# mmwillet/TTS.cpp

Hardware: AMD Instinct MI355X
Metric: audio-seconds/sec (Parler-TTS-Mini fp16, greedy decode + DAC to 44.1 kHz PCM) (higher is better)
Workload: dtype f16

## Files before the change

include/tts_hip.h:

```cpp
#ifndef TTS_HIP_H
#define TTS_HIP_H

#include <stddef.h>
#include <stdint.h>

#ifdef __cplusplus
extern "C" {
#endif

enum tts_hip_type {
    TTS_HIP_F32  = 0,
    TTS_HIP_F16  = 1,
    TTS_HIP_Q4_0 = 2,
    TTS_HIP_Q5_0 = 6,
    TTS_HIP_Q8_0 = 8,
};

#define TTS_HIP_MAX_DAC_BLOCKS 8

typedef struct tts_hip_desc {
    uint32_t struct_size;
    uint32_t hidden_size;
    uint32_t n_layers;
    uint32_t n_attn_heads;
// ... 213 lines not shown
} tts_hip_snac_desc;
tts_hip_ctx *tts_hip_snac_create(int device, const tts_hip_snac_desc *desc);
int tts_hip_snac_decode(tts_hip_ctx *ctx, const uint32_t *codes, uint32_t T, const float *noise, float *pcm_out);
int tts_hip_snac_halo_frames(const tts_hip_snac_desc *desc);
int tts_hip_snac_decode_windows(tts_hip_ctx *ctx, const uint32_t *codes, const uint32_t *frames, const uint32_t *keep0, const uint32_t *keep1, uint32_t n,
                                const float *noise, float *pcm_out);
int tts_hip_snac_decode_windows_begin(tts_hip_ctx *ctx, const uint32_t *codes, const uint32_t *frames, const uint32_t *keep0, const uint32_t *keep1, uint32_t n,
                                      const float *noise, float *pcm_out);
int tts_hip_snac_decode_windows_end(tts_hip_ctx *ctx);

int tts_hip_dac_decode(tts_hip_ctx *ctx, const uint32_t *codes, uint32_t frames, float *pcm_out);
int tts_hip_dac_decode_batch(tts_hip_ctx *ctx, const uint32_t *codes, const uint32_t *frames, uint32_t n, float *pcm_out);
int tts_hip_dac_halo_frames(const tts_hip_desc *desc);
int tts_hip_dac_decode_windows(tts_hip_ctx *ctx, const uint32_t *codes, const uint32_t *frames, const uint32_t *keep0, const uint32_t *keep1,
                               uint32_t n, float *pcm_out);

int64_t tts_hip_debug_read(tts_hip_ctx *ctx, const char *what, float *out, size_t max_floats);
int     tts_hip_set_debug(tts_hip_ctx *ctx, int on);

enum tts_hip_kclass {
    TTS_HIP_K_EMBED = 0,
    TTS_HIP_K_LN = 1,
    TTS_HIP_K_GEMM_QKV = 2,
    TTS_HIP_K_ATTN_SELF = 3,
    TTS_HIP_K_GEMM_ATTN_OUT = 4,
    TTS_HIP_K_GEMM_CROSS_Q = 5,
    TTS_HIP_K_ATTN_CROSS = 6,
    TTS_HIP_K_GEMM_CROSS_OUT = 7,
    TTS_HIP_K_GEMM_FC1 = 8,
    TTS_HIP_K_GEMM_FC2 = 9,
// ... 39 lines not shown
```

tts.cpp_amd/csrc/shim_codec.hip:

```cpp
#include "shim_internal.h"

#include "dac_kernels.h"
#include "dac_b3_kernels.h"
#include "kokoro_kernels.h"

static int dac_snapshot(tts_hip_ctx *c, int stage, const float *dev, size_t C, size_t L, size_t LS) {
    if (!c->debug) return 0;
    HIPCHK(hipStreamSynchronize(c->stream));
    std::vector<float> &v = c->dac_dbg[stage];
    v.resize(C * L);
    HIPCHK(hipMemcpy2DAsync(v.data(), L * 4, dev, LS * 4, L * 4, C, hipMemcpyDeviceToHost, c->stream));
    HIPCHK(hipStreamSynchronize(c->stream));
    return 0;
}

#define CI32_K1 16
#ifndef CI32_T
#define CI32_T 8
#endif
#ifndef CI32_K7
#define CI32_K7 4
#endif
static int conv_tile(int cout, int K, int *CO_T, int *CI_T) {
    if (K != 7 && K != 1) return -1;
// ... 509 lines not shown
    ResUnitArgs a{};
    a.x = x; a.y = y; a.w = c->packed_ru.at(r.in_w);
    a.b7 = (const float *) (c->arena + r.in_b); a.b1 = (const float *) (c->arena + r.out_b);
    a.alpha_in = (const float *) (c->arena + r.in_alpha); a.alpha_mid = (const float *) (c->arena + r.out_alpha);
    a.L = LS; a.dil = dil; a.pad = 3 * dil; a.frames = bt.frames; a.mult = bt.mult;
    const double Lv = bt.tot_frames * bt.mult;
    CHK(prof_begin(c, TTS_HIP_K_DAC_RESUNIT, (2.0 * C * Lv + 8.0 * C * C) * 4, 2.0 * C * (double) C * 8 * Lv));
    if (c->dac_tap7) {
        if (C == 96) CHK((launch_resunit_t7<3, 3>(c, a, bt.n)));
        else CHK((launch_resunit_t7<6, 4>(c, a, bt.n)));
    } else if (C == 96) CHK((launch_resunit_t<3, 4, 3>(c, a, bt.n)));
    else CHK((launch_resunit_t<6, 2, 4>(c, a, bt.n)));
    return prof_end(c);
}

static int dac_decode_batch_on(tts_hip_ctx *c, const uint32_t *codes, const uint32_t *frames, uint32_t n, float *pcm_out);
static int dac_decode_batch(tts_hip_ctx *c, const uint32_t *codes, const uint32_t *frames, uint32_t n, float *pcm_out) {
    if (!c || !c->finalized || !c->has_dac) return set_err("tts_hip_dac_decode: context has no finalized DAC");
    if (!frames || !codes || !pcm_out) return set_err("tts_hip_dac_decode: null argument");
    const uint32_t G = (uint32_t) std::max(1, c->dac_group);
    size_t code_off = 0, pcm_off = 0;
    for (uint32_t g0 = 0; g0 < n; g0 += G) {
        const uint32_t m = std::min(G, n - g0);
        size_t fr = 0;
        for (uint32_t i = 0; i < m; i++) fr += frames[g0 + i];
        int rc;
        {
            std::lock_guard<std::mutex> lock(g_dac_pass_mutex[(unsigned) c->device % 64]);
            if (!c->dac_stream) {
                rc = dac_decode_batch_on(c, codes + code_off * c->d_ncb, frames + g0, m, pcm_out + pcm_off);
            } else {
                hipStream_t ar = c->stream;
                c->stream = c->dac_stream;
                rc = dac_decode_batch_on(c, codes + code_off * c->d_ncb, frames + g0, m, pcm_out + pcm_off);
                if (rc) (void) hipStreamSynchronize(c->stream);
                c->stream = ar;
            }
            if (rc) (void) hipStreamSynchronize(c->stream);
        }
        if (rc) return rc;
        code_off += fr;
        pcm_off += fr * (size_t) c->d_up;
    }
    return 0;
}

static int dac_decode_batch_on(tts_hip_ctx *c, const uint32_t *codes, const uint32_t *frames, uint32_t n, float *pcm_out) {
    if (!c->weights_present) return set_err("tts_hip_dac_decode: weights not present");
    if (!codes || !pcm_out || !frames) return set_err("tts_hip_dac_decode: null argument");
    HIPCHK(hipSetDevice(c->device));
    uint32_t Fmax = 0;
    size_t tot = 0;
    for (uint32_t i = 0; i < n; i++) {
        if (frames[i] > c->d.dac_max_frames) return set_err("tts_hip_dac_decode: %u frames > max %u", frames[i], c->d.dac_max_frames);
        Fmax = std::max(Fmax, frames[i]);
        tot += frames[i];
    }
    if (Fmax == 0) return 0;
    for (size_t i = 0; i < tot * c->d_ncb; i++)
        if (codes[i] >= (uint32_t) c->d_cbsize) return set_err("tts_hip_dac_decode: code %u >= codebook size %d", codes[i], c->d_cbsize);
    c->dac_dbg.clear();
    CHK(ensure_packed(c));
    const size_t need_frames = (size_t) n * Fmax;
    size_t need_elems = 0, pcm_elems = 0;
    {
        int Lq = (int) Fmax;
        need_elems = (size_t) std::max(c->d_latent, c->d_c0) * dac_row_stride(c, Lq);
        if (c->packed_p.count(c->d_initw)) need_elems = std::max(need_elems, ((size_t) c->d_latent * dac_row_stride(c, Lq) * 3 + 1) / 2);
        for (auto &b : c->dblocks) {
            need_elems = std::max(need_elems, (size_t) b.cin * dac_row_stride(c, Lq));
            Lq = (Lq - 1) * b.stride - 2 * b.padding + 2 * b.stride;
            need_elems = std::max(need_elems, (size_t) b.cout * dac_row_stride(c, Lq));
            if (c->packed_p.count(b.res[0].in_w)) need_elems = std::max(need_elems, ((size_t) b.cout * dac_row_stride(c, Lq) * 3 + 1) / 2);
        }
        need_elems *= n;
        pcm_elems = (size_t) n * dac_row_stride(c, Lq);
    }
    DacBuffers &B = g_dac_buffers[(unsigned) c->device % 64];
    if (!c->dac_buf_user) { c->dac_buf_user = true; B.users++; }
    if (need_frames * c->d_ncb > B.cap_codes || need_elems > B.dbuf_elems || pcm_elems > B.h_pcm_elems || (!c->packed_p.empty() && !B.dplanes)) {
        HIPCHK(hipStreamSynchronize(c->stream));
        const size_t want_elems = std::max(need_elems, B.dbuf_elems), want_codes = std::max(need_frames * c->d_ncb, B.cap_codes), want_pcm = std::max(pcm_elems, B.h_pcm_elems);
        auto drop = [&]() {
            for (int i = 0; i < 3; i++) { free_dev(B.dbuf[i]); B.dbuf[i] = nullptr; }
            free_dev(B.dplanes); B.dplanes = nullptr;
            free_dev(B.d_codes); B.d_codes = nullptr;
            if (B.h_pcm) { (void) hipHostFree(B.h_pcm); B.h_pcm = nullptr; }
            B.dbuf_elems = B.cap_codes = B.h_pcm_elems = 0;
        };
        drop();
        hipError_t e = hipSuccess;
        for (int i = 0; i < 3 && e == hipSuccess; i++) e = hipMalloc((void **) &B.dbuf[i], want_elems * 4);
        if (e == hipSuccess && !c->packed_p.empty()) e = hipMalloc((void **) &B.dplanes, want_elems * 4);
        if (e == hipSuccess) e = hipMalloc((void **) &B.d_codes, want_codes * 4);
        if (e == hipSuccess) e = hipHostMalloc((void **) &B.h_pcm, want_pcm * 4);
        if (e != hipSuccess) {
            drop();
            return set_err("tts_hip_dac_decode: codec buffers of %zu floats x %d + %zu ids: %s", want_elems, c->packed_p.empty() ? 3 : 4, want_codes, hipGetErrorString(e));
        }
        B.dbuf_elems = want_elems; B.cap_codes = want_codes; B.h_pcm_elems = want_pcm;
    }
    if (n > c->d_frames_cap) {
        free_dev(c->d_frames);
        HIPCHK(hipMalloc((void **) &c->d_frames, (size_t) n * 4));
        c->d_frames_cap = n;
    }
    HIPCHK(hipMemcpyAsync(c->d_frames, frames, (size_t) n * 4, hipMemcpyHostToDevice, c->stream));
    {
        size_t off = 0;
        for (uint32_t i = 0; i < n; i++) {
            if (frames[i]) HIPCHK(hipMemcpyAsync(B.d_codes + (size_t) i * Fmax * c->d_ncb, codes + off * c->d_ncb, (size_t) frames[i] * c->d_ncb * 4,
                                                 hipMemcpyHostToDevice, c->stream));
            off += frames[i];
        }
    }
    DacBatch bt;
    bt.n = (int) n; bt.frames = c->d_frames; bt.mult = 1; bt.tot_frames = (double) tot;
    int L = (int) Fmax;
    int LS = dac_row_stride(c, L);
    float *cur = B.dbuf[0], *t1 = B.dbuf[1], *t2 = B.dbuf[2];

    DacEmbedArgs ea{};
    ea.frames = c->d_frames;
    ea.codes = B.d_codes; ea.codebook = (const float *) (c->arena + c->d_codebook); ea.proj_w = (const float *) (c->arena + c->d_projw);
    ea.proj_b = (const float *) (c->arena + c->d_projb); ea.n_cb = c->d_ncb; ea.cb_size = c->d_cbsize; ea.cb_dim = c->d_cbdim;
    ea.latent = c->d_latent; ea.T = L; ea.Tout = LS; ea.out = cur; ea.x_f16 = c->dac_f16 ? 1 : 0;
    CHK(prof_begin(c, TTS_HIP_K_DAC_EMBED, (double) c->d_latent * tot * 4, 2.0 * c->d_latent * tot * c->d_ncb * c->d_cbdim));
    if (c->d_ncb == 9 && c->d_cbdim == 8)
        hipLaunchKernelGGL((dac_embed_tile_kernel<9, 8>), dim3((L + 63) / 64, (c->d_latent + 4 * EMB_CH - 1) / (4 * EMB_CH), n), dim3(256), 0, c->stream, ea);
    else
// ... 58 lines not shown
        for (int r = 0; r < 3; r++) {
            int dil = 1;
            for (int e = 0; e < r; e++) dil *= 3;
            if (resunit_fused(c, b.res[r], dil)) {
                CHK(launch_resunit(c, bt, b.res[r], C, LS, dil, cur, t1));
                std::swap(cur, t1);
                continue;
            }
            CHK(launch_conv(c, bt, cur, C, LS, b.res[r].in_w, b.res[r].in_b, b.res[r].in_alpha, true, C, 7, 3 * dil, dil, nullptr, false, t1,
                            b.res[r].out_alpha, true));
            CHK(launch_conv(c, bt, t1, C, LS, b.res[r].out_w, b.res[r].out_b, 0, false, C, 1, 0, 1, cur, false, t2));
            std::swap(cur, t2);
        }
        if (n == 1) CHK(dac_snapshot(c, 2 + (int) bi, cur, (size_t) C, (size_t) L, (size_t) LS));
    }
    CHK(launch_conv(c, bt, cur, C, LS, c->d_fw, c->d_fb, c->d_falpha, true, 1, 7, 3, 1, nullptr, true, t1));
    HIPCHK(hipMemcpyAsync(B.h_pcm, t1, (size_t) n * LS * 4, hipMemcpyDeviceToHost, c->stream));
    HIPCHK(hipStreamSynchronize(c->stream));
    size_t off = 0;
    for (uint32_t i = 0; i < n; i++) {
        memcpy(pcm_out + off, B.h_pcm + (size_t) i * LS, (size_t) frames[i] * c->d_up * 4);
        off += (size_t) frames[i] * c->d_up;
    }
    return 0;
}

extern "C" int tts_hip_dac_decode(tts_hip_ctx *c, const uint32_t *codes, uint32_t frames, float *pcm_out) {
    return dac_decode_batch(c, codes, &frames, 1, pcm_out);
}

extern "C" int tts_hip_dac_decode_batch(tts_hip_ctx *c, const uint32_t *codes, const uint32_t *frames, uint32_t n, float *pcm_out) {
    if (n == 0) return 0;
    return dac_decode_batch(c, codes, frames, n, pcm_out);
}

static int64_t floor_div(int64_t a, int64_t b) { return a >= 0 ? a / b : -((-a + b - 1) / b); }

extern "C" int tts_hip_dac_halo_frames(const tts_hip_desc *d) {
    if (!d) return set_err("tts_hip_dac_halo_frames: null desc");
// ... 841 lines not shown
```

tts.cpp_amd/csrc/shim_core.hip:

```cpp
#include "shim_internal.h"

static thread_local char g_err[1024] = "";
int set_err(const char *fmt, ...) {
    va_list ap;
    va_start(ap, fmt);
    vsnprintf(g_err, sizeof(g_err), fmt, ap);
    va_end(ap);
    return -1;
}

extern "C" const char *tts_hip_last_error(void) { return g_err; }
extern "C" const char *tts_hip_version(void) { return "tts_hip 0.1 (gfx950)"; }

static float h2f_host(uint16_t h) {
    const uint32_t sign = (uint32_t) (h & 0x8000u) << 16;
    uint32_t exp = (h >> 10) & 0x1F, man = h & 0x3FF, bits;
    if (exp == 0) {
        if (man == 0) bits = sign;
        else {
            exp = 113;
            while ((man & 0x400) == 0) { man <<= 1; exp--; }
            bits = sign | (exp << 23) | ((man & 0x3FF) << 13);
        }
    } else if (exp == 31) bits = sign | 0x7F800000u | (man << 13);
// ... 151 lines not shown
    else if (k == "b1_fc2_split") c->b1_fc2_split = v != 0;
    else if (k == "b1_defer_combine") c->b1_defer_combine = v != 0;
    else if (k == "b1_stamps") c->b1_stamps_want = v != 0;
    else return set_err("tts_hip_tune: unknown key '%s'", key);
    return 0;
}

void free_dev(void *p) { if (p) (void) hipFree(p); }
std::mutex g_dac_pass_mutex[64];
static void dac_buffers_release(tts_hip_ctx *c) {
    if (!c->dac_buf_user) return;
    std::lock_guard<std::mutex> lock(g_dac_pass_mutex[(unsigned) c->device % 64]);
    DacBuffers &B = g_dac_buffers[(unsigned) c->device % 64];
    c->dac_buf_user = false;
    if (--B.users > 0) return;
    for (int i = 0; i < 3; i++) { free_dev(B.dbuf[i]); B.dbuf[i] = nullptr; }
    free_dev(B.dplanes); B.dplanes = nullptr;
    free_dev(B.d_codes); B.d_codes = nullptr;
    if (B.h_pcm) { (void) hipHostFree(B.h_pcm); B.h_pcm = nullptr; }
    B.dbuf_elems = B.cap_codes = B.h_pcm_elems = 0;
    B.users = 0;
}

static std::mutex g_arena_mutex;
static std::map<void *, int> g_arena_refs;
void arena_own(tts_hip_ctx *c) { std::lock_guard<std::mutex> l(g_arena_mutex); g_arena_refs[c->arena] = 1; }
void arena_share(tts_hip_ctx *c) {
    std::lock_guard<std::mutex> l(g_arena_mutex);
    auto it = g_arena_refs.find(c->arena);
    c->arena_counted = it != g_arena_refs.end();
    if (c->arena_counted) it->second++;
}
void arena_release(tts_hip_ctx *c) {
    if (!c->arena) return;
    if (c->arena_external && !c->arena_counted) return;
// ... 21 lines not shown
                     c->di_xn, c->di_qkv, c->di_q, c->di_att, c->di_gu, c->di_g, c->di_parts, c->di_logits, c->di_guided})
        free_dev(p);
    for (uint32_t *p : {c->di_tok, c->di_epos, c->di_eseq, c->di_kbeg, c->di_kend, c->di_ids, c->di_pos, c->di_seq, c->di_cend, c->di_stok, c->di_loop, c->di_hist, c->di_look, c->di_sbud, c->di_sadm}) free_dev(p);
    free_dev(c->di_suni);
    free_dev(c->di_e16);
    for (int i = 0; i < 3; i++) free_dev(c->sbuf[i]);
    free_dev(c->s_in); free_dev(c->s_out);
    if (c->h_in) (void) hipHostFree(c->h_in);
    if (c->h_out) (void) hipHostFree(c->h_out);
    if (c->h_hist) (void) hipHostFree(c->h_hist);
    free_dev(c->ls.state); free_dev(c->ls.tokens); free_dev(c->ls.smp); free_dev(c->ls.uni); free_dev(c->ls.cand); free_dev(c->ls.total);
    if (c->ls.h_state) (void) hipHostFree(c->ls.h_state);
    free_dev(c->t5_bucket); free_dev(c->t5_x); free_dev(c->t5_qkv); free_dev(c->t5_att); free_dev(c->t5_ug); free_dev(c->t5_g); free_dev(c->t5_y); free_dev(c->t5_ids); free_dev(c->logits); free_dev(c->part); free_dev(c->attn_cnt); free_dev(c->b1_stamps); free_dev(c->dbg); free_dev(c->d_ids); free_dev(c->d_pos);
    free_dev(c->d_seq); free_dev(c->d_gather); free_dev(c->d_tok); free_dev(c->d_step); free_dev(c->d_steps_done); free_dev(c->d_tokens_out);
    free_dev(c->d_eos); free_dev(c->d_frames);
    dac_buffers_release(c);
    for (auto &pw : c->packed) free_dev(pw.second);
    for (auto &pw : c->packed16) free_dev(pw.second);
    for (auto &pw : c->packed_b3) free_dev(pw.second);
    free_dev(c->cond_text_enc); free_dev(c->cond_cross_kv);
    for (auto &pw : c->packed_ru) free_dev(pw.second);
    for (auto &pw : c->packed_ct) free_dev(pw.second);
    for (auto &pw : c->packed_p) free_dev(pw.second);
    if (c->h_ids) (void) hipHostFree(c->h_ids);
    if (c->h_pos) (void) hipHostFree(c->h_pos);
    if (c->h_seq) (void) hipHostFree(c->h_seq);
    if (c->h_tok) (void) hipHostFree(c->h_tok);
    if (c->h_logits) (void) hipHostFree(c->h_logits);
    if (c->h_di) (void) hipHostFree(c->h_di);
    if (c->h_di_look) (void) hipHostFree(c->h_di_look);
// ... 654 lines not shown
```

tts.cpp_amd/csrc/shim_internal.h:

```cpp
#pragma once
#include "../../include/tts_hip.h"

#include <hip/hip_runtime.h>

#include <algorithm>
#include <atomic>
#include <cmath>
#include <cstdarg>
#include <cstdio>
#include <cstdlib>
#include <cstring>
#include <map>
#include <set>
#include <mutex>
#include <string>
#include <vector>

#include <unordered_map>
#define LLAMA_GREEDY_CHUNK 8

int set_err(const char *fmt, ...);
#define HIPCHK(expr)                                                                          \
    do {                                                                                      \
        hipError_t _e = (expr);                                                               \
// ... 39 lines not shown
struct DRes { size_t in_alpha, in_w, in_b, out_alpha, out_w, out_b; };
struct DBlock { int stride, padding, cin, cout; size_t alpha, w, b; DRes res[3]; };

struct CopyItem { size_t dst; std::string src; size_t src_off = 0; size_t bytes = 0; };

struct ProfEv { hipEvent_t a, b; int kclass; };

constexpr int GRAPH_KEY_ROWS = 8192;

struct DacBuffers {
    float *dbuf[3] = {nullptr, nullptr, nullptr};
    size_t dbuf_elems = 0;
    size_t cap_codes = 0;
    float *dplanes = nullptr;
    uint32_t *d_codes = nullptr;
    float *h_pcm = nullptr;
    size_t h_pcm_elems = 0;
    int users = 0;
};
extern DacBuffers g_dac_buffers[64];
extern std::mutex g_dac_pass_mutex[64];

struct tts_hip_ctx {
    int device = 0;
    hipStream_t stream = nullptr;
    hipStream_t dac_stream = nullptr;
    tts_hip_desc d{};
    std::map<std::string, Tensor> tensors;
    bool planned = false, finalized = false, weights_present = false;
    bool has_parler = false, has_dac = false;

    char *arena = nullptr;
    size_t arena_bytes = 0;
    bool arena_external = false;
// ... 182 lines not shown
        std::vector<uint32_t> start, row_utt;
    } gl;
    int gen_total = 0;
    bool gen_compact = true;
    uint32_t *d_tokens_out = nullptr;
    size_t tokens_out_cap = 0;
    uint8_t *d_eos = nullptr;
    uint32_t *h_ids = nullptr, *h_pos = nullptr, *h_seq = nullptr, *h_tok = nullptr;
    float *h_logits = nullptr;
    std::vector<uint32_t> host_pos;

    size_t dac_frame_elems = 0;
    size_t dac_cap_frames = 0;
    uint32_t *d_frames = nullptr;
    size_t d_frames_cap = 0;
    bool debug = false;
    std::map<int, std::vector<float>> dac_dbg;
    std::vector<float> win_pcm;
    std::map<size_t, float *> packed;
    std::set<size_t> packed_direct;
    std::map<size_t, _Float16 *> packed16;
    std::map<size_t, __bf16 *> packed_b3;
    std::map<size_t, __bf16 *> packed_ru;
    std::map<size_t, __bf16 *> packed_p;
    int dac_split = 1;
    int dac_f16_planes = 1;
    int dac_tap7 = 1;
    int dac_wdma = 1;
    int dac_planes = 1;
    bool dac_buf_user = false;
// ... 97 lines not shown
```

tts.cpp_amd/hip.py:

```python
import ctypes as C
import os

import numpy as np

from . import gguf

PKG_DIR = os.path.dirname(os.path.abspath(__file__))
MAX_DAC_BLOCKS = 8

FLAG_NO_GRAPH, FLAG_VALU_GEMM, FLAG_NO_DAC, FLAG_NO_PARLER, FLAG_DEQUANT_Q, FLAG_DAC_F32 = 1, 2, 4, 8, 16, 32
KCLASSES = ["embed", "ln", "gemm_qkv", "attn_self", "gemm_attn_out", "gemm_cross_q", "attn_cross", "gemm_cross_out", "gemm_fc1",
            "gemm_fc2", "gemm_heads", "sample", "gemm_other", "dac_embed", "dac_conv7", "dac_conv1", "dac_convt", "dac_final", "dac_resunit", "kokoro_conv_mfma"]


class HipError(RuntimeError):
    pass


class Desc(C.Structure):
    _fields_ = [
        ("struct_size", C.c_uint32),
        ("hidden_size", C.c_uint32), ("n_layers", C.c_uint32), ("n_attn_heads", C.c_uint32),
        ("n_output_heads", C.c_uint32), ("output_vocab_size", C.c_uint32), ("max_ctx_length", C.c_uint32),
        ("n_encode_length", C.c_uint32), ("use_cross_attn", C.c_uint32),
# ... 35 lines not shown
        (n, C.c_float) for n in ("attn_scale", "upsample_scale", "sample_rate", "sin_amp", "noise_std", "voice_threshold")] + [
        ("up_stride", C.c_uint32 * 4), ("up_padding", C.c_uint32 * 4), ("noise_stride", C.c_uint32 * 4), ("noise_padding", C.c_uint32 * 4),
        ("res_padding", (C.c_uint32 * 3) * 16), ("res_dilation", (C.c_uint32 * 3) * 16), ("noise_res_padding", (C.c_uint32 * 3) * 4),
        ("noise_res_dilation", (C.c_uint32 * 3) * 4), ("flags", C.c_uint32)]


class KStat(C.Structure):
    _fields_ = [("ms_total", C.c_double), ("launches", C.c_uint64), ("bytes_total", C.c_double), ("flops_total", C.c_double)]


EXPORTS = [
    "tts_hip_device_count", "tts_hip_create", "tts_hip_destroy", "tts_hip_last_error", "tts_hip_version",
    "tts_hip_upload", "tts_hip_arena_bytes", "tts_hip_finalize", "tts_hip_arena_ptr", "tts_hip_arena_filled",
    "tts_hip_parler_set_text_encoding", "tts_hip_parler_reset", "tts_hip_parler_prefill", "tts_hip_parler_prefill_batch", "tts_hip_parler_step",
    "tts_hip_parler_step_greedy", "tts_hip_parler_generate_greedy", "tts_hip_parler_generate_sampled", "tts_hip_sample_logits",
    "tts_hip_t5_create", "tts_hip_t5_encode", "tts_hip_t5_output_size", "tts_hip_snac_create", "tts_hip_snac_decode", "tts_hip_orpheus_create", "tts_hip_orpheus_decode", "tts_hip_orpheus_step_batch", "tts_hip_orpheus_generate_batch", "tts_hip_orpheus_generate_greedy", "tts_hip_orpheus_generate_sampled", "tts_hip_orpheus_sample_logits", "tts_hip_dia_create", "tts_hip_dia_encode", "tts_hip_dia_step", "tts_hip_dia_encode_slot", "tts_hip_dia_step_batch", "tts_hip_dia_generate", "tts_hip_kokoro_create", "tts_hip_kokoro_durations", "tts_hip_kokoro_generate", "tts_hip_dac_decode", "tts_hip_dac_decode_batch", "tts_hip_debug_read",
    "tts_hip_set_debug", "tts_hip_profile", "tts_hip_profile_get", "tts_hip_kclass_name", "tts_hip_stream",
    "tts_hip_synchronize", "tts_hip_dac_arith", "tts_hip_broadcast_weights", "tts_hip_comm_unique_id", "tts_hip_broadcast_weights_rank", "tts_hip_tune",
    "tts_hip_parler_stream_begin", "tts_hip_parler_stream_admit", "tts_hip_parler_stream_run", "tts_hip_parler_stream_collect", "tts_hip_parler_stream_end",
    "tts_hip_parler_gen_begin", "tts_hip_parler_gen_launch", "tts_hip_parler_gen_wait", "tts_hip_dac_halo_frames", "tts_hip_dac_decode_windows",
    "tts_hip_snac_halo_frames", "tts_hip_snac_decode_windows", "tts_hip_snac_decode_windows_begin", "tts_hip_snac_decode_windows_end",
    "tts_hip_orpheus_gen_begin", "tts_hip_orpheus_gen_launch", "tts_hip_orpheus_gen_wait",
    "tts_hip_orpheus_stream_begin", "tts_hip_orpheus_stream_admit", "tts_hip_orpheus_stream_run", "tts_hip_orpheus_stream_collect", "tts_hip_orpheus_stream_end",
    "tts_hip_orpheus_sample_logits_rows",
    "tts_hip_orpheus_stream_begin_mixed", "tts_hip_orpheus_stream_admit_mixed", "tts_hip_orpheus_sample_logits_rows_mixed",
    "tts_hip_dia_gen_begin", "tts_hip_dia_gen_launch", "tts_hip_dia_gen_wait",
    "tts_hip_dia_stream_begin", "tts_hip_dia_stream_admit", "tts_hip_dia_stream_run", "tts_hip_dia_stream_collect", "tts_hip_dia_stream_end",
    "tts_hip_dia_stream_launch", "tts_hip_dia_stream_wait", "tts_hip_dia_stream_drop",
]

class Sampling(C.Structure):
# ... 59 lines not shown
    L.tts_hip_dia_create.argtypes = [C.c_int, C.POINTER(DiaDesc)]
    L.tts_hip_dia_encode.argtypes = [vp, u32p, C.c_uint32, f32p]
    L.tts_hip_dia_step.argtypes = [vp, u32p, C.c_uint32, f32p, f32p]
    L.tts_hip_dia_encode_slot.argtypes = [vp, C.c_uint32, u32p, C.c_uint32, f32p]
    L.tts_hip_dia_step_batch.argtypes = [vp, C.c_uint32, u32p, u32p, u32p, f32p, f32p]
    L.tts_hip_dia_generate.argtypes = [vp, C.c_uint32, C.c_uint32, C.POINTER(DiaCodes), C.POINTER(Sampling), f32p, u32p, u32p]
    L.tts_hip_snac_create.restype = vp
    L.tts_hip_snac_create.argtypes = [C.c_int, C.POINTER(SnacDesc)]
    L.tts_hip_snac_decode.argtypes = [vp, u32p, C.c_uint32, f32p, f32p]
    L.tts_hip_t5_create.restype = vp
    L.tts_hip_t5_create.argtypes = [C.c_int, C.POINTER(T5Desc)]
    L.tts_hip_t5_encode.argtypes = [vp, u32p, C.c_uint32, f32p]
    L.tts_hip_t5_output_size.argtypes = [vp]
    L.tts_hip_dac_decode.argtypes = [vp, u32p, C.c_uint32, f32p]
    L.tts_hip_dac_decode_batch.argtypes = [vp, u32p, u32p, C.c_uint32, f32p]
    L.tts_hip_debug_read.argtypes = [vp, C.c_char_p, f32p, C.c_size_t]
    L.tts_hip_debug_read.restype = C.c_int64
    L.tts_hip_set_debug.argtypes = [vp, C.c_int]
    L.tts_hip_profile.argtypes = [vp, C.c_int]
    L.tts_hip_profile_get.argtypes = [vp, C.c_int, C.POINTER(KStat)]
    L.tts_hip_kclass_name.argtypes = [C.c_int]
    L.tts_hip_kclass_name.restype = C.c_char_p
    L.tts_hip_stream.argtypes = [vp]
    L.tts_hip_stream.restype = vp
    L.tts_hip_synchronize.argtypes = [vp]
    L.tts_hip_tune.argtypes = [vp, C.c_char_p, C.c_int]
    L.tts_hip_parler_stream_begin.argtypes = [vp, C.c_uint32, C.c_uint32, C.c_uint32, C.c_uint32, C.POINTER(Sampling)]
    L.tts_hip_parler_stream_admit.argtypes = [vp, C.c_uint32, u32p, u32p, u32p, f32p]
    L.tts_hip_parler_stream_run.argtypes = [vp, C.c_uint32, u32p, u32p, u32p]
    L.tts_hip_parler_stream_collect.argtypes = [vp, C.c_uint32, C.c_uint32, u32p]
# ... 927 lines not shown
```

tts.cpp_amd/host/parler_runner.cpp:

```cpp
#include "parler_runner.h"

#include <algorithm>
#include <cstdlib>
#include <cstring>

#include "gguf.h"

parler_model_loader::parler_model_loader() : tts_model_loader{"parler-tts"} {}
const parler_model_loader parler_loader{};
void parler_register() {}

static parler_hparams read_hparams(const gguf_file & m) {
    parler_hparams hp;
    if (!m.get_u32({"parler-tts.decoder.encode_length", "encode_length"}, hp.n_encode_length))
        TTS_ABORT("key 'parler-tts.decoder.encode_length' must be specified in gguf file.\n");
    m.get_u32({"parler-tts.decoder.hidden_size", "hidden_size"}, hp.hidden_size);
    m.get_u32({"parler-tts.decoder.output_heads", "output_heads"}, hp.n_output_heads);
    m.get_u32({"parler-tts.decoder.context_length", "ctx_length"}, hp.max_ctx_length);
    m.get_u32({"parler-tts.decoder.attention.head_count", "attn_heads"}, hp.n_attn_heads);
    m.get_u32({"parler-tts.decoder.out_vocab_size", "out_vocab_size"}, hp.output_vocab_size);
    m.get_u32({"parler-tts.decoder.audio_vocab_size", "audio_vocab_size"}, hp.audio_vocab_size);
    m.get_u32({"parler-tts.decoder.max_generation", "max_generation"}, hp.max_generation_size);
    m.get_u32({"parler-tts.decoder.num_hidden_layers", "num_hidden_layers"}, hp.n_layers);
    m.get_u32({"audio.bos_token_id", "bos_token_id"}, hp.bos_token_id);
// ... 343 lines not shown
                go = hook->emit();
            }
        }
    }
    if (hook && go) {
        finished.assign(n, true);
        hook->plan(toks, finished);
        (void) hook->emit();
    }
    return toks;
}

std::vector<tts_response> parler_runner::decode_frames(const std::vector<uint32_t> & codes, const std::vector<uint32_t> & frames) {
    size_t total = 0;
    for (uint32_t f : frames) total += (size_t) f * hp.up_sampling_factor;
    pcm.assign(total, 0.0f);
    if (total) hip_check(tts_hip_dac_decode_batch(ctx, codes.data(), frames.data(), (uint32_t) frames.size(), pcm.data()), "tts_hip_dac_decode_batch");
    std::vector<tts_response> audio(frames.size());
    size_t off = 0;
    for (size_t i = 0; i < frames.size(); i++) {
        audio[i].data = pcm.data() + off;
        audio[i].n_outputs = (size_t) frames[i] * hp.up_sampling_factor;
        off += audio[i].n_outputs;
    }
    return audio;
}

void parler_runner::generate(const char * sentence, tts_response & output, const generation_configuration & config) {
    std::vector<uint32_t> prompt, codes;
    output.data = nullptr;
    output.n_outputs = 0;
// ... 152 lines not shown
```

Measured before the change: 995.3.

## Double-buffer DAC codec passes so a pass launches before the previous is collected

Replaces the synchronous per-group DAC decode with a two-slot pass ring. Each group's codes and frame counts are staged into a pinned host image. PCM goes to per-slot device and pinned host buffers, with an event per slot. A caller can enqueue the next group's kernels while the previous pass's PCM is still being copied back and unpacked, and it releases the shared pass lock sooner so other callers can hand over faster. The cost is more device and pinned memory, plus a more complex locking and slot lifecycle that needs its own test harness. The runner also stops zero-filling the PCM buffer on every call.

Measured after the change: 997.3, median of 4. About the same (+0.2%).

```diff
diff --git a/include/tts_hip.h b/include/tts_hip.h
--- a/include/tts_hip.h
+++ b/include/tts_hip.h
@@ -251,6 +251,8 @@
 int tts_hip_dac_halo_frames(const tts_hip_desc *desc);
 int tts_hip_dac_decode_windows(tts_hip_ctx *ctx, const uint32_t *codes, const uint32_t *frames, const uint32_t *keep0, const uint32_t *keep1,
                                uint32_t n, float *pcm_out);
+
+int tts_hip_dac_passes_in_flight(int device);
 
 int64_t tts_hip_debug_read(tts_hip_ctx *ctx, const char *what, float *out, size_t max_floats);
 int     tts_hip_set_debug(tts_hip_ctx *ctx, int on);
diff --git a/profiles/codec_pass_gap.py b/profiles/codec_pass_gap.py
--- /dev/null
+++ b/profiles/codec_pass_gap.py
@@ -0,0 +1,69 @@
+#!/usr/bin/env python3
+import bisect
+import csv
+import json
+import sys
+
+CODEC = ("resunit", "conv_b3p", "convt_b3", "conv1d", "convt1d", "snake_split", "dac_embed", "conv1x1")
+HANDOVER_MS = 40.0
+
+rows = []
+for r in csv.DictReader(open(sys.argv[1])):
+    rows.append((int(r["Start_Timestamp"]), int(r["End_Timestamp"]), r["Kernel_Name"]))
+rows.sort()
+t0, t1 = rows[0][0], rows[-1][1]
+lo, hi = t0 + (t1 - t0) * 0.35, t0 + (t1 - t0) * 0.95
+rows = [r for r in rows if r[0] >= lo and r[1] <= hi]
+
+busy = []
+for s, e, _ in rows:
+    if busy and s <= busy[-1][1]:
+        busy[-1][1] = max(busy[-1][1], e)
+    else:
+        busy.append([s, e])
+bstart = [b[0] for b in busy]
+
+
+def busy_in(a, b):
+    t = 0
+    k = max(0, bisect.bisect_right(bstart, a) - 1)
+    while k < len(busy) and busy[k][0] < b:
+        t += max(0, min(b, busy[k][1]) - max(a, busy[k][0]))
+        k += 1
+    return t
+
+
+codec = [(s, e, n) for s, e, n in rows if any(k in n for k in CODEC)]
+cstart = [s for s, _, _ in codec]
+finals = [(s, e) for s, e, n in codec if "conv1d_cout1" in n]
+gaps = []
+for s, e in finals:
+    k = bisect.bisect_left(cstart, e)
+    if k >= len(codec):
+        continue
+    nxt = codec[k][0]
+    gaps.append(((nxt - e) / 1e6, (nxt - e - busy_in(e, nxt)) / 1e6))
+span = (rows[-1][1] - rows[0][0]) / 1e6
+hand = sorted(g for g in gaps if g[0] <= HANDOVER_MS)
+away = [g for g in gaps if g[0] > HANDOVER_MS]
+
+
+def pct(v, p):
+    return round(v[min(len(v) - 1, int(p * len(v)))], 3) if v else None
+
+
+hg = [g[0] for g in hand]
+out = {
+    "label": sys.argv[2] if len(sys.argv) > 2 else "",
+    "window_ms": round(span, 1),
+    "passes": len(finals),
+    "handover_gaps": {"count": len(hand), "limit_ms": HANDOVER_MS, "median_ms": pct(hg, 0.5), "p10_ms": pct(hg, 0.1), "p90_ms": pct(hg, 0.9),
+                      "max_ms": round(max(hg), 3) if hg else None, "sum_ms": round(sum(hg), 2),
+                      "sum_no_kernel_running_ms": round(sum(g[1] for g in hand), 2),
+                      "no_kernel_share_of_gap": round(sum(g[1] for g in hand) / max(sum(hg), 1e-9), 3),
+                      "gap_share_of_window": round(sum(hg) / span, 4),
+                      "no_kernel_share_of_window": round(sum(g[1] for g in hand) / span, 4)},
+    "longer_gaps": {"count": len(away), "sum_ms": round(sum(g[0] for g in away), 1), "sum_no_kernel_running_ms": round(sum(g[1] for g in away), 1)},
+    "any_kernel_running_share_of_window": round(sum(b[1] - b[0] for b in busy) / 1e6 / span, 4),
+}
+print(json.dumps(out))
diff --git a/tts.cpp_amd/csrc/dac_pass_ring.h b/tts.cpp_amd/csrc/dac_pass_ring.h
--- /dev/null
+++ b/tts.cpp_amd/csrc/dac_pass_ring.h
@@ -0,0 +1,74 @@
+#pragma once
+#include <condition_variable>
+#include <cstdint>
+#include <mutex>
+
+template <class Event, int N = 2>
+class PassRing {
+public:
+    static constexpr int kSlots = N;
+
+    int take(bool block) {
+        std::unique_lock<std::mutex> l(mu_);
+        for (;;) {
+            int best = -1;
+            for (int s = 0; s < N; s++)
+                if (slot_[s].state == FREE && (best < 0 || slot_[s].freed_at < slot_[best].freed_at)) best = s;
+            if (best >= 0) { slot_[best].state = TAKEN; return best; }
+            if (!block) return -1;
+            cv_.wait(l);
+        }
+    }
+    void launched(int s, Event done) {
+        std::lock_guard<std::mutex> l(mu_);
+        slot_[s].done = done;
+        slot_[s].state = IN_FLIGHT;
+    }
+    void abandon(int s) { free_slot(s); }
+    void set_last_kernels(Event e) { std::lock_guard<std::mutex> l(mu_); last_ = e; has_last_ = true; }
+    bool last_kernels(Event *e) { std::lock_guard<std::mutex> l(mu_); if (has_last_) *e = last_; return has_last_; }
+    void forget_last_kernels() { std::lock_guard<std::mutex> l(mu_); has_last_ = false; }
+
+    template <class Wait>
+    bool wait_done(int s, Wait &&wait, int *rc) {
+        Event e;
+        {
+            std::lock_guard<std::mutex> l(mu_);
+            if (s < 0 || s >= N || slot_[s].state != IN_FLIGHT) return false;
+            e = slot_[s].done;
+        }
+        *rc = wait(e);
+        std::lock_guard<std::mutex> l(mu_);
+        slot_[s].state = DONE;
+        return true;
+    }
+    bool release(int s) {
+        {
+            std::lock_guard<std::mutex> l(mu_);
+            if (s < 0 || s >= N || slot_[s].state != DONE) return false;
+        }
+        free_slot(s);
+        return true;
+    }
+
+    void wait_idle() {
+        std::unique_lock<std::mutex> l(mu_);
+        cv_.wait(l, [&] { return busy_locked() == 0; });
+    }
+    int in_flight() { std::lock_guard<std::mutex> l(mu_); return busy_locked(); }
+
+private:
+    enum State { FREE, TAKEN, IN_FLIGHT, DONE };
+    struct Slot { State state = FREE; Event done{}; uint64_t freed_at = 0; };
+    int busy_locked() const { int n = 0; for (int s = 0; s < N; s++) n += slot_[s].state != FREE; return n; }
+    void free_slot(int s) {
+        { std::lock_guard<std::mutex> l(mu_); slot_[s].state = FREE; slot_[s].freed_at = ++clock_; }
+        cv_.notify_all();
+    }
+    std::mutex mu_;
+    std::condition_variable cv_;
+    Slot slot_[N];
+    uint64_t clock_ = 0;
+    Event last_{};
+    bool has_last_ = false;
+};
diff --git a/tts.cpp_amd/csrc/shim_codec.hip b/tts.cpp_amd/csrc/shim_codec.hip
--- a/tts.cpp_amd/csrc/shim_codec.hip
+++ b/tts.cpp_amd/csrc/shim_codec.hip
@@ -547,41 +547,31 @@
     return prof_end(c);
 }
 
-static int dac_decode_batch_on(tts_hip_ctx *c, const uint32_t *codes, const uint32_t *frames, uint32_t n, float *pcm_out);
-static int dac_decode_batch(tts_hip_ctx *c, const uint32_t *codes, const uint32_t *frames, uint32_t n, float *pcm_out) {
-    if (!c || !c->finalized || !c->has_dac) return set_err("tts_hip_dac_decode: context has no finalized DAC");
-    if (!frames || !codes || !pcm_out) return set_err("tts_hip_dac_decode: null argument");
-    const uint32_t G = (uint32_t) std::max(1, c->dac_group);
-    size_t code_off = 0, pcm_off = 0;
-    for (uint32_t g0 = 0; g0 < n; g0 += G) {
-        const uint32_t m = std::min(G, n - g0);
-        size_t fr = 0;
-        for (uint32_t i = 0; i < m; i++) fr += frames[g0 + i];
-        int rc;
-        {
-            std::lock_guard<std::mutex> lock(g_dac_pass_mutex[(unsigned) c->device % 64]);
-            if (!c->dac_stream) {
-                rc = dac_decode_batch_on(c, codes + code_off * c->d_ncb, frames + g0, m, pcm_out + pcm_off);
-            } else {
-                hipStream_t ar = c->stream;
-                c->stream = c->dac_stream;
-                rc = dac_decode_batch_on(c, codes + code_off * c->d_ncb, frames + g0, m, pcm_out + pcm_off);
-                if (rc) (void) hipStreamSynchronize(c->stream);
-                c->stream = ar;
-            }
-            if (rc) (void) hipStreamSynchronize(c->stream);
-        }
-        if (rc) return rc;
-        code_off += fr;
-        pcm_off += fr * (size_t) c->d_up;
-    }
-    return 0;
-}
-
-static int dac_decode_batch_on(tts_hip_ctx *c, const uint32_t *codes, const uint32_t *frames, uint32_t n, float *pcm_out) {
+struct DacPass {
+    int slot = -1;
+    const float *h_pcm = nullptr;
+    const uint32_t *frames = nullptr;
+    uint32_t n = 0;
+    size_t LS = 0;
+    float *out = nullptr;
+};
+struct DacStaged { const uint32_t *img = nullptr; uint32_t Fmax = 0; size_t tot = 0; };
+constexpr int DAC_COLLECT_FIRST = 1;
+
+void dac_buffers_drop(DacBuffers &B) {
+    for (int i = 0; i < 3; i++) { free_dev(B.dbuf[i]); B.dbuf[i] = nullptr; }
+    free_dev(B.dplanes); B.dplanes = nullptr;
+    free_dev(B.d_codes); B.d_codes = nullptr;
+    for (int s = 0; s < 2; s++) {
+        free_dev(B.d_pcm[s]); B.d_pcm[s] = nullptr;
+        if (B.h_pcm[s]) { (void) hipHostFree(B.h_pcm[s]); B.h_pcm[s] = nullptr; }
+    }
+    B.dbuf_elems = B.cap_codes = B.h_pcm_elems = 0;
+}
+
+static int dac_pass_stage(tts_hip_ctx *c, const uint32_t *codes, const uint32_t *frames, uint32_t n, int k, DacStaged *st) {
     if (!c->weights_present) return set_err("tts_hip_dac_decode: weights not present");
-    if (!codes || !pcm_out || !frames) return set_err("tts_hip_dac_decode: null argument");
-    HIPCHK(hipSetDevice(c->device));
+    if (!codes || !frames) return set_err("tts_hip_dac_decode: null argument");
     uint32_t Fmax = 0;
     size_t tot = 0;
     for (uint32_t i = 0; i < n; i++) {
@@ -589,11 +579,40 @@
         Fmax = std::max(Fmax, frames[i]);
         tot += frames[i];
     }
+    st->Fmax = Fmax; st->tot = tot; st->img = nullptr;
     if (Fmax == 0) return 0;
-    for (size_t i = 0; i < tot * c->d_ncb; i++)
+    const size_t ncb = (size_t) c->d_ncb;
+    for (size_t i = 0; i < tot * ncb; i++)
         if (codes[i] >= (uint32_t) c->d_cbsize) return set_err("tts_hip_dac_decode: code %u >= codebook size %d", codes[i], c->d_cbsize);
+    const size_t ids = (size_t) n + (size_t) n * Fmax * ncb;
+    if (ids > c->h_dac_in_cap[k]) {
+        HIPCHK(hipSetDevice(c->device));
+        if (c->h_dac_in[k]) { (void) hipHostFree(c->h_dac_in[k]); c->h_dac_in[k] = nullptr; c->h_dac_in_cap[k] = 0; }
+        HIPCHK(hipHostMalloc((void **) &c->h_dac_in[k], ids * 4));
+        c->h_dac_in_cap[k] = ids;
+    }
+    uint32_t *img = c->h_dac_in[k];
+    memcpy(img, frames, (size_t) n * 4);
+    size_t off = 0;
+    for (uint32_t i = 0; i < n; i++) {
+        uint32_t *row = img + n + (size_t) i * Fmax * ncb;
+        memcpy(row, codes + off * ncb, (size_t) frames[i] * ncb * 4);
+        memset(row + (size_t) frames[i] * ncb, 0, (size_t) (Fmax - frames[i]) * ncb * 4);
+        off += frames[i];
+    }
+    st->img = img;
+    return 0;
+}
+
+static int dac_pass_launch(tts_hip_ctx *c, DacBuffers &B, const DacStaged &st, uint32_t n, int slot, size_t *LS_out);
+
+static int dac_pass_enqueue(tts_hip_ctx *c, const DacStaged &st, const uint32_t *frames, uint32_t n, float *pcm_out, bool may_block, DacPass *p) {
+    *p = DacPass{};
+    if (st.Fmax == 0) return 0;
+    HIPCHK(hipSetDevice(c->device));
     c->dac_dbg.clear();
     CHK(ensure_packed(c));
+    const uint32_t Fmax = st.Fmax;
     const size_t need_frames = (size_t) n * Fmax;
     size_t need_elems = 0, pcm_elems = 0;
     {
@@ -612,41 +631,117 @@
     DacBuffers &B = g_dac_buffers[(unsigned) c->device % 64];
     if (!c->dac_buf_user) { c->dac_buf_user = true; B.users++; }
     if (need_frames * c->d_ncb > B.cap_codes || need_elems > B.dbuf_elems || pcm_elems > B.h_pcm_elems || (!c->packed_p.empty() && !B.dplanes)) {
+        if (!may_block) return DAC_COLLECT_FIRST;
+        B.ring.wait_idle();
         HIPCHK(hipStreamSynchronize(c->stream));
         const size_t want_elems = std::max(need_elems, B.dbuf_elems), want_codes = std::max(need_frames * c->d_ncb, B.cap_codes), want_pcm = std::max(pcm_elems, B.h_pcm_elems);
-        auto drop = [&]() {
-            for (int i = 0; i < 3; i++) { free_dev(B.dbuf[i]); B.dbuf[i] = nullptr; }
-            free_dev(B.dplanes); B.dplanes = nullptr;
-            free_dev(B.d_codes); B.d_codes = nullptr;
-            if (B.h_pcm) { (void) hipHostFree(B.h_pcm); B.h_pcm = nullptr; }
-            B.dbuf_elems = B.cap_codes = B.h_pcm_elems = 0;
-        };
-        drop();
+        dac_buffers_drop(B);
+        B.ring.forget_last_kernels();
         hipError_t e = hipSuccess;
+        for (int s = 0; s < 2 && e == hipSuccess; s++)
+            if (!B.slot_ev[s]) e = hipEventCreateWithFlags(&B.slot_ev[s], hipEventDisableTiming);
+        if (e == hipSuccess && !B.ev_kernels) e = hipEventCreateWithFlags(&B.ev_kernels, hipEventDisableTiming);
+        if (e == hipSuccess && !B.copy_stream) e = hipStreamCreateWithFlags(&B.copy_stream, hipStreamNonBlocking);
         for (int i = 0; i < 3 && e == hipSuccess; i++) e = hipMalloc((void **) &B.dbuf[i], want_elems * 4);
         if (e == hipSuccess && !c->packed_p.empty()) e = hipMalloc((void **) &B.dplanes, want_elems * 4);
         if (e == hipSuccess) e = hipMalloc((void **) &B.d_codes, want_codes * 4);
-        if (e == hipSuccess) e = hipHostMalloc((void **) &B.h_pcm, want_pcm * 4);
+        for (int s = 0; s < 2 && e == hipSuccess; s++) {
+            e = hipMalloc((void **) &B.d_pcm[s], want_pcm * 4);
+            if (e == hipSuccess) e = hipHostMalloc((void **) &B.h_pcm[s], want_pcm * 4);
+        }
         if (e != hipSuccess) {
-            drop();
+            dac_buffers_drop(B);
             return set_err("tts_hip_dac_decode: codec buffers of %zu floats x %d + %zu ids: %s", want_elems, c->packed_p.empty() ? 3 : 4, want_codes, hipGetErrorString(e));
         }
         B.dbuf_elems = want_elems; B.cap_codes = want_codes; B.h_pcm_elems = want_pcm;
     }
     if (n > c->d_frames_cap) {
         free_dev(c->d_frames);
+        c->d_frames = nullptr; c->d_frames_cap = 0;
         HIPCHK(hipMalloc((void **) &c->d_frames, (size_t) n * 4));
         c->d_frames_cap = n;
     }
-    HIPCHK(hipMemcpyAsync(c->d_frames, frames, (size_t) n * 4, hipMemcpyHostToDevice, c->stream));
-    {
+    const int slot = B.ring.take(may_block);
+    if (slot < 0) return DAC_COLLECT_FIRST;
+    size_t LS = 0;
+    const int rc = dac_pass_launch(c, B, st, n, slot, &LS);
+    if (rc) {
+        (void) hipStreamSynchronize(c->stream);
+        (void) hipStreamSynchronize(B.copy_stream);
+        B.ring.abandon(slot);
+        return rc;
+    }
+    B.ring.launched(slot, B.slot_ev[slot]);
+    p->slot = slot; p->h_pcm = B.h_pcm[slot]; p->frames = frames; p->n = n; p->LS = LS; p->out = pcm_out;
+    return 0;
+}
+
+static int dac_pass_collect(tts_hip_ctx *c, DacPass *p) {
+    if (p->slot < 0) return 0;
+    DacBuffers &B = g_dac_buffers[(unsigned) c->device % 64];
+    const int slot = p->slot;
+    p->slot = -1;
+    int werr = 0;
+    if (!B.ring.wait_done(slot, [](hipEvent_t e) { return (int) hipEventSynchronize(e); }, &werr)) return set_err("tts_hip_dac_decode: pass slot %d is not in flight", slot);
+    if (werr == 0) {
         size_t off = 0;
-        for (uint32_t i = 0; i < n; i++) {
-            if (frames[i]) HIPCHK(hipMemcpyAsync(B.d_codes + (size_t) i * Fmax * c->d_ncb, codes + off * c->d_ncb, (size_t) frames[i] * c->d_ncb * 4,
-                                                 hipMemcpyHostToDevice, c->stream));
-            off += frames[i];
-        }
-    }
+        for (uint32_t i = 0; i < p->n; i++) {
+            memcpy(p->out + off, p->h_pcm + (size_t) i * p->LS, (size_t) p->frames[i] * c->d_up * 4);
+            off += (size_t) p->frames[i] * c->d_up;
+        }
+    }
+    B.ring.release(slot);
+    if (werr) return set_err("tts_hip_dac_decode: waiting for the pass: %s", hipGetErrorString((hipError_t) werr));
+    return 0;
+}
+
+static int dac_decode_batch(tts_hip_ctx *c, const uint32_t *codes, const uint32_t *frames, uint32_t n, float *pcm_out) {
+    if (!c || !c->finalized || !c->has_dac) return set_err("tts_hip_dac_decode: context has no finalized DAC");
+    if (!frames || !codes || !pcm_out) return set_err("tts_hip_dac_decode: null argument");
+    const uint32_t G = (uint32_t) std::max(1, c->dac_group);
+    size_t code_off = 0, pcm_off = 0;
+    DacPass pend;
+    int rc = 0;
+    for (uint32_t g0 = 0; g0 < n && rc == 0; g0 += G) {
+        const uint32_t m = std::min(G, n - g0);
+        size_t fr = 0;
+        for (uint32_t i = 0; i < m; i++) fr += frames[g0 + i];
+        DacStaged st;
+        rc = dac_pass_stage(c, codes + code_off * c->d_ncb, frames + g0, m, (int) (c->dac_pass_no++ & 1), &st);
+        DacPass cur;
+        while (rc == 0) {
+            {
+                std::unique_lock<std::mutex> lock(g_dac_pass_mutex[(unsigned) c->device % 64], std::defer_lock);
+                if (pend.slot >= 0 && !lock.try_lock()) {
+                    if ((rc = dac_pass_collect(c, &pend)) != 0) break;
+                }
+                if (!lock.owns_lock()) lock.lock();
+                hipStream_t ar = c->stream;
+                if (c->dac_stream) c->stream = c->dac_stream;
+                rc = dac_pass_enqueue(c, st, frames + g0, m, pcm_out + pcm_off, pend.slot < 0, &cur);
+                if (rc == 0 && c->debug) rc = dac_pass_collect(c, &cur);
+                c->stream = ar;
+            }
+            if (rc != DAC_COLLECT_FIRST) break;
+            rc = dac_pass_collect(c, &pend);
+        }
+        const int prc = dac_pass_collect(c, &pend);
+        if (rc == 0) rc = prc;
+        pend = cur;
+        code_off += fr;
+        pcm_off += fr * (size_t) c->d_up;
+    }
+    const int prc = dac_pass_collect(c, &pend);
+    return rc ? rc : prc;
+}
+
+static int dac_pass_launch(tts_hip_ctx *c, DacBuffers &B, const DacStaged &st, uint32_t n, int slot, size_t *LS_out) {
+    const uint32_t Fmax = st.Fmax;
+    const size_t tot = st.tot;
+    hipEvent_t before;
+    if (B.ring.last_kernels(&before)) HIPCHK(hipStreamWaitEvent(c->stream, before, 0));
+    HIPCHK(hipMemcpyAsync(c->d_frames, st.img, (size_t) n * 4, hipMemcpyHostToDevice, c->stream));
+    HIPCHK(hipMemcpyAsync(B.d_codes, st.img + n, (size_t) n * Fmax * c->d_ncb * 4, hipMemcpyHostToDevice, c->stream));
     DacBatch bt;
     bt.n = (int) n; bt.frames = c->d_frames; bt.mult = 1; bt.tot_frames = (double) tot;
     int L = (int) Fmax;
@@ -735,15 +830,19 @@
         }
         if (n == 1) CHK(dac_snapshot(c, 2 + (int) bi, cur, (size_t) C, (size_t) L, (size_t) LS));
     }
-    CHK(launch_conv(c, bt, cur, C, LS, c->d_fw, c->d_fb, c->d_falpha, true, 1, 7, 3, 1, nullptr, true, t1));
-    HIPCHK(hipMemcpyAsync(B.h_pcm, t1, (size_t) n * LS * 4, hipMemcpyDeviceToHost, c->stream));
-    HIPCHK(hipStreamSynchronize(c->stream));
-    size_t off = 0;
-    for (uint32_t i = 0; i < n; i++) {
-        memcpy(pcm_out + off, B.h_pcm + (size_t) i * LS, (size_t) frames[i] * c->d_up * 4);
-        off += (size_t) frames[i] * c->d_up;
-    }
-    return 0;
+    CHK(launch_conv(c, bt, cur, C, LS, c->d_fw, c->d_fb, c->d_falpha, true, 1, 7, 3, 1, nullptr, true, B.d_pcm[slot]));
+    HIPCHK(hipEventRecord(B.ev_kernels, c->stream));
+    B.ring.set_last_kernels(B.ev_kernels);
+    HIPCHK(hipStreamWaitEvent(B.copy_stream, B.ev_kernels, 0));
+    HIPCHK(hipMemcpyAsync(B.h_pcm[slot], B.d_pcm[slot], (size_t) n * LS * 4, hipMemcpyDeviceToHost, B.copy_stream));
+    HIPCHK(hipEventRecord(B.slot_ev[slot], B.copy_stream));
+    *LS_out = (size_t) LS;
+    return 0;
+}
+
+extern "C" int tts_hip_dac_passes_in_flight(int device) {
+    if (device < 0 || device >= 64) return -1;
+    return g_dac_buffers[device].ring.in_flight();
 }
 
 extern "C" int tts_hip_dac_decode(tts_hip_ctx *c, const uint32_t *codes, uint32_t frames, float *pcm_out) {
diff --git a/tts.cpp_amd/csrc/shim_core.hip b/tts.cpp_amd/csrc/shim_core.hip
--- a/tts.cpp_amd/csrc/shim_core.hip
+++ b/tts.cpp_amd/csrc/shim_core.hip
@@ -189,11 +189,12 @@
     DacBuffers &B = g_dac_buffers[(unsigned) c->device % 64];
     c->dac_buf_user = false;
     if (--B.users > 0) return;
-    for (int i = 0; i < 3; i++) { free_dev(B.dbuf[i]); B.dbuf[i] = nullptr; }
-    free_dev(B.dplanes); B.dplanes = nullptr;
-    free_dev(B.d_codes); B.d_codes = nullptr;
-    if (B.h_pcm) { (void) hipHostFree(B.h_pcm); B.h_pcm = nullptr; }
-    B.dbuf_elems = B.cap_codes = B.h_pcm_elems = 0;
+    B.ring.wait_idle();
+    B.ring.forget_last_kernels();
+    dac_buffers_drop(B);
+    for (int s = 0; s < 2; s++) if (B.slot_ev[s]) { (void) hipEventDestroy(B.slot_ev[s]); B.slot_ev[s] = nullptr; }
+    if (B.ev_kernels) { (void) hipEventDestroy(B.ev_kernels); B.ev_kernels = nullptr; }
+    if (B.copy_stream) { (void) hipStreamDestroy(B.copy_stream); B.copy_stream = nullptr; }
     B.users = 0;
 }
 
@@ -245,6 +246,7 @@
     free_dev(c->t5_bucket); free_dev(c->t5_x); free_dev(c->t5_qkv); free_dev(c->t5_att); free_dev(c->t5_ug); free_dev(c->t5_g); free_dev(c->t5_y); free_dev(c->t5_ids); free_dev(c->logits); free_dev(c->part); free_dev(c->attn_cnt); free_dev(c->b1_stamps); free_dev(c->dbg); free_dev(c->d_ids); free_dev(c->d_pos);
     free_dev(c->d_seq); free_dev(c->d_gather); free_dev(c->d_tok); free_dev(c->d_step); free_dev(c->d_steps_done); free_dev(c->d_tokens_out);
     free_dev(c->d_eos); free_dev(c->d_frames);
+    for (int k = 0; k < 2; k++) if (c->h_dac_in[k]) (void) hipHostFree(c->h_dac_in[k]);
     dac_buffers_release(c);
     for (auto &pw : c->packed) free_dev(pw.second);
     for (auto &pw : c->packed16) free_dev(pw.second);
diff --git a/tts.cpp_amd/csrc/shim_internal.h b/tts.cpp_amd/csrc/shim_internal.h
--- a/tts.cpp_amd/csrc/shim_internal.h
+++ b/tts.cpp_amd/csrc/shim_internal.h
@@ -2,6 +2,8 @@
 #include "../../include/tts_hip.h"
 
 #include <hip/hip_runtime.h>
+
+#include "dac_pass_ring.h"
 
 #include <algorithm>
 #include <atomic>
@@ -77,10 +79,15 @@
     size_t cap_codes = 0;
     float *dplanes = nullptr;
     uint32_t *d_codes = nullptr;
-    float *h_pcm = nullptr;
+    float *d_pcm[2] = {nullptr, nullptr};
+    float *h_pcm[2] = {nullptr, nullptr};
     size_t h_pcm_elems = 0;
+    hipEvent_t slot_ev[2] = {nullptr, nullptr}, ev_kernels = nullptr;
+    hipStream_t copy_stream = nullptr;
+    PassRing<hipEvent_t, 2> ring;
     int users = 0;
 };
+void dac_buffers_drop(DacBuffers &B);
 extern DacBuffers g_dac_buffers[64];
 extern std::mutex g_dac_pass_mutex[64];
 
@@ -293,6 +300,9 @@
     size_t dac_cap_frames = 0;
     uint32_t *d_frames = nullptr;
     size_t d_frames_cap = 0;
+    uint32_t *h_dac_in[2] = {nullptr, nullptr};
+    size_t h_dac_in_cap[2] = {0, 0};
+    unsigned dac_pass_no = 0;
     bool debug = false;
     std::map<int, std::vector<float>> dac_dbg;
     std::vector<float> win_pcm;
diff --git a/tts.cpp_amd/hip.py b/tts.cpp_amd/hip.py
--- a/tts.cpp_amd/hip.py
+++ b/tts.cpp_amd/hip.py
@@ -73,7 +73,7 @@
     "tts_hip_upload", "tts_hip_arena_bytes", "tts_hip_finalize", "tts_hip_arena_ptr", "tts_hip_arena_filled",
     "tts_hip_parler_set_text_encoding", "tts_hip_parler_reset", "tts_hip_parler_prefill", "tts_hip_parler_prefill_batch", "tts_hip_parler_step",
     "tts_hip_parler_step_greedy", "tts_hip_parler_generate_greedy", "tts_hip_parler_generate_sampled", "tts_hip_sample_logits",
-    "tts_hip_t5_create", "tts_hip_t5_encode", "tts_hip_t5_output_size", "tts_hip_snac_create", "tts_hip_snac_decode", "tts_hip_orpheus_create", "tts_hip_orpheus_decode", "tts_hip_orpheus_step_batch", "tts_hip_orpheus_generate_batch", "tts_hip_orpheus_generate_greedy", "tts_hip_orpheus_generate_sampled", "tts_hip_orpheus_sample_logits", "tts_hip_dia_create", "tts_hip_dia_encode", "tts_hip_dia_step", "tts_hip_dia_encode_slot", "tts_hip_dia_step_batch", "tts_hip_dia_generate", "tts_hip_kokoro_create", "tts_hip_kokoro_durations", "tts_hip_kokoro_generate", "tts_hip_dac_decode", "tts_hip_dac_decode_batch", "tts_hip_debug_read",
+    "tts_hip_t5_create", "tts_hip_t5_encode", "tts_hip_t5_output_size", "tts_hip_snac_create", "tts_hip_snac_decode", "tts_hip_orpheus_create", "tts_hip_orpheus_decode", "tts_hip_orpheus_step_batch", "tts_hip_orpheus_generate_batch", "tts_hip_orpheus_generate_greedy", "tts_hip_orpheus_generate_sampled", "tts_hip_orpheus_sample_logits", "tts_hip_dia_create", "tts_hip_dia_encode", "tts_hip_dia_step", "tts_hip_dia_encode_slot", "tts_hip_dia_step_batch", "tts_hip_dia_generate", "tts_hip_kokoro_create", "tts_hip_kokoro_durations", "tts_hip_kokoro_generate", "tts_hip_dac_decode", "tts_hip_dac_decode_batch", "tts_hip_dac_passes_in_flight", "tts_hip_debug_read",
     "tts_hip_set_debug", "tts_hip_profile", "tts_hip_profile_get", "tts_hip_kclass_name", "tts_hip_stream",
     "tts_hip_synchronize", "tts_hip_dac_arith", "tts_hip_broadcast_weights", "tts_hip_comm_unique_id", "tts_hip_broadcast_weights_rank", "tts_hip_tune",
     "tts_hip_parler_stream_begin", "tts_hip_parler_stream_admit", "tts_hip_parler_stream_run", "tts_hip_parler_stream_collect", "tts_hip_parler_stream_end",
@@ -163,6 +163,8 @@
     L.tts_hip_t5_output_size.argtypes = [vp]
     L.tts_hip_dac_decode.argtypes = [vp, u32p, C.c_uint32, f32p]
     L.tts_hip_dac_decode_batch.argtypes = [vp, u32p, u32p, C.c_uint32, f32p]
+    L.tts_hip_dac_passes_in_flight.argtypes = [C.c_int]
+    L.tts_hip_dac_passes_in_flight.restype = C.c_int
     L.tts_hip_debug_read.argtypes = [vp, C.c_char_p, f32p, C.c_size_t]
     L.tts_hip_debug_read.restype = C.c_int64
     L.tts_hip_set_debug.argtypes = [vp, C.c_int]
diff --git a/tts.cpp_amd/host/parler_runner.cpp b/tts.cpp_amd/host/parler_runner.cpp
--- a/tts.cpp_amd/host/parler_runner.cpp
+++ b/tts.cpp_amd/host/parler_runner.cpp
@@ -381,7 +381,7 @@
 std::vector<tts_response> parler_runner::decode_frames(const std::vector<uint32_t> & codes, const std::vector<uint32_t> & frames) {
     size_t total = 0;
     for (uint32_t f : frames) total += (size_t) f * hp.up_sampling_factor;
-    pcm.assign(total, 0.0f);
+    if (pcm.size() < total) pcm.resize(total);
     if (total) hip_check(tts_hip_dac_decode_batch(ctx, codes.data(), frames.data(), (uint32_t) frames.size(), pcm.data()), "tts_hip_dac_decode_batch");
     std::vector<tts_response> audio(frames.size());
     size_t off = 0;
diff --git a/tts.cpp_amd/host/ring_check.cpp b/tts.cpp_amd/host/ring_check.cpp
--- /dev/null
+++ b/tts.cpp_amd/host/ring_check.cpp
@@ -0,0 +1,141 @@
+#include "../csrc/dac_pass_ring.h"
+
+#include <atomic>
+#include <cstdio>
+#include <cstdlib>
+#include <deque>
+#include <memory>
+#include <thread>
+#include <vector>
+
+struct FakeEvent {
+    std::atomic<bool> done{false};
+    std::mutex mu;
+    std::condition_variable cv;
+    void complete() { { std::lock_guard<std::mutex> l(mu); done.store(true); } cv.notify_all(); }
+    int wait() { std::unique_lock<std::mutex> l(mu); cv.wait(l, [&] { return done.load(); }); return 0; }
+};
+
+static std::atomic<int> g_failures{0};
+#define EXPECT(cond, ...) do { if (!(cond)) { g_failures++; fprintf(stderr, "ring_check: " __VA_ARGS__); fputc('\n', stderr); } } while (0)
+
+struct Job { FakeEvent *ev; int slot; long id; };
+struct Device {
+    std::mutex mu;
+    std::condition_variable cv;
+    std::deque<Job> q;
+    bool stop = false;
+    std::atomic<long> staging[2];
+    void push(Job j) { { std::lock_guard<std::mutex> l(mu); q.push_back(j); } cv.notify_one(); }
+    void run() {
+        for (;;) {
+            Job j;
+            {
+                std::unique_lock<std::mutex> l(mu);
+                cv.wait(l, [&] { return stop || !q.empty(); });
+                if (q.empty()) return;
+                j = q.front(); q.pop_front();
+            }
+            std::this_thread::yield();
+            staging[j.slot].store(j.id);
+            j.ev->complete();
+        }
+    }
+};
+
+struct Shared {
+    PassRing<FakeEvent *, 2> ring;
+    std::mutex pass_lock;
+    Device dev;
+    FakeEvent *last_ev[2] = {nullptr, nullptr};
+    std::atomic<int> owner[2];
+    std::atomic<int> in_flight{0}, max_in_flight{0};
+};
+
+struct Pass { int slot = -1; long id = 0; };
+
+static void collect(Shared &S, int me, Pass *p, std::vector<long> *collected) {
+    if (p->slot < 0) return;
+    int rc = -1;
+    const bool ok = S.ring.wait_done(p->slot, [](FakeEvent *e) { return e->wait(); }, &rc);
+    EXPECT(ok && rc == 0, "caller %d: wait_done(slot %d) refused", me, p->slot);
+    EXPECT(S.dev.staging[p->slot].load() == p->id, "caller %d: slot %d holds pass %ld, not %ld: handed on before it was collected", me, p->slot, S.dev.staging[p->slot].load(), p->id);
+    collected->push_back(p->id);
+    S.owner[p->slot].store(-1);
+    S.in_flight--;
+    EXPECT(S.ring.release(p->slot), "caller %d: release(slot %d) refused", me, p->slot);
+    p->slot = -1;
+}
+
+static void caller(Shared &S, int me, int calls, int groups, std::vector<std::unique_ptr<FakeEvent>> *events) {
+    std::vector<long> enqueued, collected;
+    long next = (long) me * 1000000;
+    for (int call = 0; call < calls; call++) {
+        Pass pend;
+        for (int g = 0; g < groups; g++) {
+            Pass cur;
+            for (;;) {
+                std::unique_lock<std::mutex> lock(S.pass_lock, std::defer_lock);
+                if (pend.slot >= 0 && !lock.try_lock()) collect(S, me, &pend, &collected);
+                if (!lock.owns_lock()) lock.lock();
+                const bool may_block = pend.slot < 0;
+                if (may_block && (call * groups + g) % 7 == 3) {
+                    S.ring.wait_idle();
+                    EXPECT(S.ring.in_flight() == 0 && S.in_flight.load() == 0, "caller %d: ring not idle after wait_idle", me);
+                }
+                const int s = S.ring.take(may_block);
+                if (s < 0) {
+                    EXPECT(!may_block, "caller %d: a blocking take returned no slot", me);
+                    lock.unlock();
+                    collect(S, me, &pend, &collected);
+                    continue;
+                }
+                EXPECT(S.owner[s].load() == -1, "caller %d: slot %d handed out while caller %d still owns it", me, s, S.owner[s].load());
+                EXPECT(!S.last_ev[s] || S.last_ev[s]->done.load(), "caller %d: slot %d handed out before its previous event completed", me, s);
+                const int now = ++S.in_flight;
+                int seen = S.max_in_flight.load();
+                while (now > seen && !S.max_in_flight.compare_exchange_weak(seen, now)) {}
+                EXPECT(now <= 2 && S.ring.in_flight() <= 2, "caller %d: %d passes in flight", me, now);
+                S.owner[s].store(me);
+                events->emplace_back(new FakeEvent);
+                FakeEvent *ev = events->back().get();
+                S.last_ev[s] = ev;
+                cur.slot = s; cur.id = ++next;
+                S.ring.set_last_kernels(ev);
+                S.dev.push({ev, s, cur.id});
+                S.ring.launched(s, ev);
+                enqueued.push_back(cur.id);
+                break;
+            }
+            collect(S, me, &pend, &collected);
+            pend = cur;
+        }
+        collect(S, me, &pend, &collected);
+    }
+    EXPECT(enqueued == collected, "caller %d: collect order differs from enqueue order (%zu enqueued, %zu collected)", me, enqueued.size(), collected.size());
+    EXPECT((int) enqueued.size() == calls * groups, "caller %d: %zu passes, expected %d", me, enqueued.size(), calls * groups);
+}
+
+int main(int argc, char **argv) {
+    const int calls = argc > 1 ? atoi(argv[1]) : 200, groups = 5, T = 3;
+    Shared S;
+    for (int s = 0; s < 2; s++) { S.owner[s].store(-1); S.dev.staging[s].store(-1); }
+    std::thread device([&] { S.dev.run(); });
+    std::vector<std::vector<std::unique_ptr<FakeEvent>>> events(T);
+    std::vector<std::thread> th;
+    for (int t = 0; t < T; t++) th.emplace_back(caller, std::ref(S), t, calls, groups, &events[t]);
+    for (auto &t : th) t.join();
+    { std::lock_guard<std::mutex> l(S.dev.mu); S.dev.stop = true; }
+    S.dev.cv.notify_all();
+    device.join();
+    EXPECT(S.ring.in_flight() == 0, "passes left in flight at the end");
+    int rc = 0;
+    EXPECT(!S.ring.release(0), "release of a free slot accepted");
+    EXPECT(!S.ring.wait_done(1, [](FakeEvent *) { return 0; }, &rc), "wait_done on a free slot accepted");
+    const int s = S.ring.take(false);
+    EXPECT(s >= 0 && !S.ring.release(s), "release of a slot nobody waited for accepted");
+    S.ring.abandon(s);
+    EXPECT(S.ring.in_flight() == 0, "abandon did not free the slot");
+    printf("ring_check: %d callers x %d calls x %d passes, at most %d in flight, %d failures\n", T, calls, groups, S.max_in_flight.load(), g_failures.load());
+    return g_failures.load() ? 1 : 0;
+}
```
